# hmmlillian/Neural-Color-Transfer

Hardware: AMD Instinct MI355X
Metric: 700x700 pairs/sec end-to-end L=5->1; PatchMatch HBM GB/s vs peak (higher is better)
Workload: dtype f32

## Files before the change

### neural-color-transfer_amd/csrc/k_s1.hip

```cpp
#include "nct_internal.h"
#include "nct_device.h"
#include "nct_reduce.h"
#include <rocprim/device/device_radix_sort.hpp>
#include <rocprim/device/device_scan.hpp>

#define LAB_D(u) ((double)(u) * (1.0 / 255.0))
#define LCHK() NCT_LAUNCH_CHECK()

constexpr int S1_SEG = NCT_S1_SEG;

struct S1Sys {
    int n, h, w;
    const double *daa, *dab, *dbb;
    const double *gx, *gy;
    const int* knn_id;
    nct_s1_graph g;
    int xcd;
    int one_xcd;
};
__device__ __forceinline__ int s1_one_xcd(int bid, int sel) { return (bid & 7) == sel - 1 ? (bid >> 3) : -1; }
__device__ __forceinline__ int s1_block_of(int bid, int nblocks, int xcd) {
    if (!xcd) return bid;
    const int q = nblocks >> 3, r = nblocks & 7, x = bid & 7, idx = bid >> 3;
    return (x < r ? x * (q + 1) : r * (q + 1) + (x - r) * q) + idx;
// ... 164 lines not shown
constexpr int S1_CHUNK = 1024;
template <bool COOP>
__device__ __forceinline__ void s1_op(const S1Sys& S, const double* __restrict__ p, int i, bool live, double (&a)[3], double (&b)[3], double (&ya)[3], double (&yb)[3], int lb = -1) {
    const int w = S.w, h = S.h;
    int e0 = 0, e1 = 0, h0 = 0, h1 = 0;
#pragma unroll
    for (int c = 0; c < 3; ++c) { a[c] = 0.0; b[c] = 0.0; ya[c] = 0.0; yb[c] = 0.0; }
    if (live) {
        const int y = i / w, x = i - y * w;
        { double own[6]; ld6(p, (size_t)i, own);
#pragma unroll
          for (int c = 0; c < 3; ++c) { a[c] = own[c]; b[c] = own[3 + c]; } }
#pragma unroll
        for (int c = 0; c < 3; ++c) {
            ya[c] = S.daa[(size_t)i * 3 + c] * a[c] + S.dab[(size_t)i * 3 + c] * b[c];
            yb[c] = S.dab[(size_t)i * 3 + c] * a[c] + S.dbb[(size_t)i * 3 + c] * b[c];
        }
        auto edge = [&](int j, double wt) {
            double q[6]; ld6(p, (size_t)j, q);
#pragma unroll
            for (int c = 0; c < 3; ++c) { ya[c] += wt * (a[c] - q[c]); yb[c] += wt * (b[c] - q[3 + c]); }
        };
        {
            const bool ex[4] = {x + 1 < w, x > 0, y + 1 < h, y > 0};
            const int nj[4] = {ex[0] ? i + 1 : i, ex[1] ? i - 1 : i, ex[2] ? i + w : i, ex[3] ? i - w : i};
            const double g4[4] = {S.gx[i], S.gx[ex[1] ? i - 1 : i], S.gy[i], S.gy[ex[3] ? i - w : i]};
            double q4[4][6];
#pragma unroll
            for (int u = 0; u < 4; ++u) ld6(p, (size_t)nj[u], q4[u]);
#pragma unroll
            for (int u = 0; u < 4; ++u)
                if (ex[u]) {
                    const double wt = 2.0 * (g4[u] * g4[u]);
#pragma unroll
                    for (int c = 0; c < 3; ++c) { ya[c] += wt * (a[c] - q4[u][c]); yb[c] += wt * (b[c] - q4[u][3 + c]); }
                }
        }
#pragma unroll
        for (int k = 0; k < 8; ++k) edge(S.knn_id[(size_t)i * 8 + k], S.g.iw2[(size_t)i * 8 + k]);
        const unsigned long long s0 = S.g.starts[i], s1 = S.g.starts[i + 1];
        e0 = lo32(s0); e1 = lo32(s1); h0 = hi32(s0); h1 = hi32(s1);
    }
    if constexpr (!COOP) {
        if (live) {
            int e = e0;
            for (; e + 4 <= e1; e += 4) {
                int j[4]; double wt[4], pv[4][6];
#pragma unroll
                for (int u = 0; u < 4; ++u) { j[u] = S.g.c_src[e + u]; wt[u] = S.g.c_w[e + u]; }
#pragma unroll
                for (int u = 0; u < 4; ++u) ld6(p, (size_t)j[u], pv[u]);
#pragma unroll
                for (int u = 0; u < 4; ++u)
#pragma unroll
                    for (int c = 0; c < 3; ++c) { ya[c] += wt[u] * (a[c] - pv[u][c]); yb[c] += wt[u] * (b[c] - pv[u][3 + c]); }
            }
            for (; e < e1; ++e) {
                const int j = S.g.c_src[e]; const double wt = S.g.c_w[e];
                double q[6]; ld6(p, (size_t)j, q);
#pragma unroll
                for (int c = 0; c < 3; ++c) { ya[c] += wt * (a[c] - q[c]); yb[c] += wt * (b[c] - q[3 + c]); }
            }
        }
    } else {
        __shared__ double s_pv[6 * S1_CHUNK];
        __shared__ double s_wt[S1_CHUNK];
        const int i0 = (lb >= 0 ? lb : (int)blockIdx.x) * 256, i1 = min(i0 + 256, S.n);
        const int E0 = lo32(S.g.starts[i0]), E1 = lo32(S.g.starts[i1]);
        for (int base = E0; base < E1; base += S1_CHUNK) {
            const int cnt = min(S1_CHUNK, E1 - base);
            for (int t = threadIdx.x; t < cnt; t += 256) {
                const int j = S.g.c_src[base + t];
                s_wt[t] = S.g.c_w[base + t];
                double q[6]; ld6(p, (size_t)j, q);
#pragma unroll
                for (int c = 0; c < 6; ++c) s_pv[c * S1_CHUNK + t] = q[c];
            }
            __syncthreads();
            const int lo = max(e0, base) - base, hi = min(e1, base + cnt) - base;
            for (int t = lo; t < hi; ++t) {
                const double wt = s_wt[t];
#pragma unroll
                for (int c = 0; c < 3; ++c) { ya[c] += wt * (a[c] - s_pv[c * S1_CHUNK + t]); yb[c] += wt * (b[c] - s_pv[(3 + c) * S1_CHUNK + t]); }
            }
            __syncthreads();
        }
    }
    bool sup = false;
    if (h1 - h0 > S1_SEG) { h0 = S.g.sup_start[i]; h1 = S.g.sup_start[i + 1]; sup = true; }
    const double* __restrict__ part = sup ? S.g.sup_part : S.g.hub_part;
    for (int sg = h0; sg < h1; ++sg) {
        double q[6]; ld6(part, (size_t)sg, q);
#pragma unroll
        for (int c = 0; c < 3; ++c) { ya[c] += q[c]; yb[c] += q[3 + c]; }
    }
}

template <bool COOP>
__global__ __launch_bounds__(256) void k_s1_residual(S1Sys S, const double* __restrict__ x6, const double* __restrict__ rhs, double* __restrict__ r6) {
    const int i = blockIdx.x * 256 + threadIdx.x;
    double a[3], b[3], ya[3], yb[3];
    s1_op<COOP>(S, x6, i, i < S.n, a, b, ya, yb);
    if (i < S.n) {
        double o[6];
#pragma unroll
        for (int c = 0; c < 3; ++c) { o[c] = rhs[(size_t)i * 3 + c] - ya[c]; o[3 + c] = rhs[(size_t)(S.n + i) * 3 + c] - yb[c]; }
        st6(r6, (size_t)i, o);
    }
}
template <bool COOP>
__global__ __launch_bounds__(256) void k_s1_apply(S1Sys S, const double* __restrict__ r6, double* __restrict__ w6, double* __restrict__ partial ) {
    const int lb = S.one_xcd ? s1_one_xcd(blockIdx.x, S.one_xcd) : s1_block_of(blockIdx.x, gridDim.x, S.xcd);
    if (lb < 0) return;
    const int i = lb * 256 + threadIdx.x;
    double acc[6] = {0, 0, 0, 0, 0, 0};
    double a[3], b[3], ya[3], yb[3];
    s1_op<COOP>(S, r6, i, i < S.n, a, b, ya, yb, lb);
    if (i < S.n) {
#pragma unroll
        for (int c = 0; c < 3; ++c) {
            acc[c] = a[c] * a[c] + b[c] * b[c];
            acc[3 + c] = a[c] * ya[c] + b[c] * yb[c];
        }
        const double o[6] = {ya[0], ya[1], ya[2], yb[0], yb[1], yb[2]};
        st6(w6, (size_t)i, o);
    }
    block_reduce_store<6>(acc, partial, lb);
}

__device__ __forceinline__ void s1_scalars(bool first, const double (&sm)[6], const S1State* __restrict__ in, double tol2, S1State& o) {
#pragma unroll
    for (int c = 0; c < 3; ++c) {
        if (first) {
            const double g0 = sm[c]; const bool act = g0 > tol2;
            o.gm[c] = g0; o.be[c] = 0.0; o.al[c] = act ? g0 / sm[3 + c] : 0.0; o.active[c] = act ? 1 : 0; o.iters[c] = act ? 1 : 0;
        } else if (in->active[c]) {
            const double g1 = sm[c];
            const double be = g1 / in->gm[c];
            const double al = g1 / (sm[3 + c] - (be * g1) / in->al[c]);
            const bool act = g1 > tol2;
            o.gm[c] = g1; o.be[c] = be; o.al[c] = al; o.active[c] = act ? 1 : 0; o.iters[c] = in->iters[c] + (act ? 1 : 0);
        } else {
            o.gm[c] = in->gm[c]; o.be[c] = in->be[c]; o.al[c] = in->al[c]; o.active[c] = 0; o.iters[c] = in->iters[c];
        }
    }
}
__global__ __launch_bounds__(256) void k_s1_scal(const double* __restrict__ partial, int nb, const S1State* __restrict__ in, S1State* __restrict__ out, int first, double tol2) {
    double sm[6]; final_reduce<6>(partial, nb, sm);
    if (threadIdx.x == 0) { S1State o; s1_scalars(first != 0, sm, in, tol2, o); *out = o; }
}
constexpr int S1_FUSE_NB = 512;
template <bool FUSED>
__global__ __launch_bounds__(256) void k_s1_update(int n, int nb, const double* __restrict__ partial, const S1State* __restrict__ sin, S1State* __restrict__ sout,
                                                   int first_scal, double tol2, int first_vec, double* __restrict__ r6, const double* __restrict__ w6,
                                                   double* __restrict__ p6, double* __restrict__ s6, double* __restrict__ x6, int one_xcd) {
    const int bid = one_xcd ? s1_one_xcd(blockIdx.x, one_xcd) : (int)blockIdx.x;
    if (bid < 0) return;
    const size_t total = (size_t)3 * n;
    const size_t base = (size_t)bid * 768 + threadIdx.x;
    double2 rv[3], wv[3], pv[3], sv[3], xv[3];
    const double2* r2 = reinterpret_cast<const double2*>(r6); const double2* w2 = reinterpret_cast<const double2*>(w6);
    const double2* x2 = reinterpret_cast<const double2*>(x6); const double2* p2 = reinterpret_cast<const double2*>(p6); const double2* s2 = reinterpret_cast<const double2*>(s6);
#pragma unroll
    for (int k = 0; k < 3; ++k) {
        const size_t g0 = base + (size_t)k * 256, g = g0 < total ? g0 : total - 1;
        rv[k] = r2[g]; wv[k] = w2[g]; xv[k] = x2[g];
        pv[k] = p2[g]; sv[k] = s2[g];
        if (first_vec) { pv[k] = make_double2(0.0, 0.0); sv[k] = make_double2(0.0, 0.0); }
    }
    double al[3], be[3]; bool act[3];
    if constexpr (FUSED) {
        double sm[6]; final_reduce<6>(partial, nb, sm);
        S1State o; s1_scalars(first_scal != 0, sm, sin, tol2, o);
        if (bid == 0 && threadIdx.x == 0) *sout = o;
#pragma unroll
        for (int c = 0; c < 3; ++c) { al[c] = o.al[c]; be[c] = o.be[c]; act[c] = o.active[c] != 0; }
    } else {
#pragma unroll
        for (int c = 0; c < 3; ++c) { al[c] = sin->al[c]; be[c] = sin->be[c]; act[c] = sin->active[c] != 0; }
    }
    double2* r2o = reinterpret_cast<double2*>(r6); double2* x2o = reinterpret_cast<double2*>(x6); double2* p2o = reinterpret_cast<double2*>(p6); double2* s2o = reinterpret_cast<double2*>(s6);
#pragma unroll
    for (int k = 0; k < 3; ++k) {
        const size_t g = base + (size_t)k * 256;
        if (g >= total) continue;
        const int c0 = (int)((2 * g) % 3), c1 = (c0 + 1) % 3;
        const double a0 = c0 == 0 ? al[0] : (c0 == 1 ? al[1] : al[2]), b0 = c0 == 0 ? be[0] : (c0 == 1 ? be[1] : be[2]);
        const double a1 = c1 == 0 ? al[0] : (c1 == 1 ? al[1] : al[2]), b1 = c1 == 0 ? be[0] : (c1 == 1 ? be[1] : be[2]);
        const bool on0 = c0 == 0 ? act[0] : (c0 == 1 ? act[1] : act[2]), on1 = c1 == 0 ? act[0] : (c1 == 1 ? act[1] : act[2]);
        double2 pn, sn, xn, rn;
        pn.x = first_vec ? rv[k].x : b0 * pv[k].x + rv[k].x;  pn.y = first_vec ? rv[k].y : b1 * pv[k].y + rv[k].y;
        sn.x = first_vec ? wv[k].x : b0 * sv[k].x + wv[k].x;  sn.y = first_vec ? wv[k].y : b1 * sv[k].y + wv[k].y;
        xn.x = xv[k].x + a0 * pn.x;  xn.y = xv[k].y + a1 * pn.y;
        rn.x = rv[k].x - a0 * sn.x;  rn.y = rv[k].y - a1 * sn.y;
        if (!on0) { pn.x = pv[k].x; sn.x = sv[k].x; xn.x = xv[k].x; rn.x = rv[k].x; }
        if (!on1) { pn.y = pv[k].y; sn.y = sv[k].y; xn.y = xv[k].y; rn.y = rv[k].y; }
        if (on0 || on1) { p2o[g] = pn; s2o[g] = sn; x2o[g] = xn; r2o[g] = rn; }
    }
}
__global__ void k_pack6(int n, const double* __restrict__ x, double* __restrict__ x6) {
    const int i = blockIdx.x * blockDim.x + threadIdx.x;
    if (i >= 2 * n * 3) return;
    const int c = i % 3, part = i / (n * 3), px = (i - part * n * 3) / 3;
    x6[(size_t)px * 6 + part * 3 + c] = x[i];
}
__global__ void k_unpack6(int n, const double* __restrict__ x6, double* __restrict__ x) {
    const int i = blockIdx.x * blockDim.x + threadIdx.x;
    if (i >= 2 * n * 3) return;
    const int c = i % 3, part = i / (n * 3), px = (i - part * n * 3) / 3;
    x[i] = x6[(size_t)px * 6 + part * 3 + c];
}

int nctk_s1_solve(nct_ctx* ctx, hipStream_t s, const nct_s1_graph& g, const int* knn_id, const double* weight, float dWeight, const uint8_t* s_lab_level,
                  const uint8_t* g_lab_level, const double* gx, const double* gy, int layer, int h, int w, double* x, int* cg_iters_host ) {
    const int n = h * w, nbl = cdiv(n, 256);
    DevBuf<double> daa(ctx, (size_t)3 * n), dab(ctx, (size_t)3 * n), dbb(ctx, (size_t)3 * n), rhs(ctx, (size_t)6 * n);
    DevBuf<double> x6(ctx, (size_t)6 * n), r6(ctx, (size_t)6 * n), w6(ctx, (size_t)6 * n), p6(ctx, (size_t)6 * n), s6(ctx, (size_t)6 * n), partial(ctx, (size_t)nbl * 6);
    DevBuf<S1State> st(ctx, 2);
    if (!daa.ok() || !dab.ok() || !dbb.ok() || !rhs.ok() || !x6.ok() || !r6.ok() || !w6.ok() || !p6.ok() || !s6.ok() || !partial.ok() || !st.ok()) return NCT_ERR_HIP;
    hipLaunchKernelGGL(k_s1_setup, dim3(nbl), dim3(256), 0, s, n, weight, dWeight, s_lab_level, g_lab_level, (double*)daa, (double*)dab, (double*)dbb, (double*)rhs); LCHK();
    constexpr int one_xcd_max = 32;
    const int one_xcd = (nbl <= one_xcd_max && nbl <= S1_FUSE_NB) ? 1 + (ctx->home_xcd & 7) : 0;
    const int ogrid = one_xcd ? nbl * 8 : nbl;
    S1Sys S{n, h, w, daa, dab, dbb, gx, gy, knn_id, g, n >= 100000 ? 1 : 0, one_xcd};
    const double tol2 = 1e-6 * 1e-6;
    const int maxit = ctx->s1_maxit > 0 ? ctx->s1_maxit : (layer == 4 ? 50 : 100);
    const bool coop = n >= 100000;
    const bool fused = nbl <= S1_FUSE_NB;
    const int hub_blind = cdiv(cdiv(8 * n, S1_SEG), 4) < 256 ? cdiv(cdiv(8 * n, S1_SEG), 4) : 256;
    const int hub_grid = g.nseg_hint == 0 ? 0 : (g.nseg_hint > 0 ? (cdiv(g.nseg_hint, 4) < 4096 ? cdiv(g.nseg_hint, 4) : 4096) : hub_blind);
    const int hub2_grid = (g.nseg_hint == 0 || g.nsup_hint == 0) ? 0 : (g.nsup_hint > 0 ? (cdiv(g.nsup_hint, 4) < 1024 ? cdiv(g.nsup_hint, 4) : 1024) : (cdiv(hub_blind, S1_SEG) < 64 ? cdiv(hub_blind, S1_SEG) : 64));
    auto hub = [&](const double* v) -> int {
        if (hub_grid) { hipLaunchKernelGGL(k_s1_hub, dim3(hub_grid), dim3(256), 0, s, g, v); LCHK(); }
        if (hub2_grid) { hipLaunchKernelGGL(k_s1_hub2, dim3(hub2_grid), dim3(256), 0, s, g); LCHK(); }
        return 0;
    };
    auto apply = [&](bool kt) -> int {
        if (kt) NCT_TRY(ctx->kt_begin(s, NCT_KT_S1_APPLY));
        if (coop) hipLaunchKernelGGL(k_s1_apply<true>, dim3(nbl), dim3(256), 0, s, S, (const double*)r6, (double*)w6, (double*)partial);
        else      hipLaunchKernelGGL(k_s1_apply<false>, dim3(ogrid), dim3(256), 0, s, S, (const double*)r6, (double*)w6, (double*)partial);
        LCHK();
        if (kt) NCT_TRY(ctx->kt_end(s));
        return 0;
    };
    hipLaunchKernelGGL(k_pack6, dim3(cdiv(6 * n, 256)), dim3(256), 0, s, n, (const double*)x, (double*)x6); LCHK();
    NCT_TRY(hub(x6));
    if (coop) hipLaunchKernelGGL(k_s1_residual<true>, dim3(nbl), dim3(256), 0, s, S, (const double*)x6, (const double*)rhs, (double*)r6);
    else      hipLaunchKernelGGL(k_s1_residual<false>, dim3(nbl), dim3(256), 0, s, S, (const double*)x6, (const double*)rhs, (double*)r6);
    LCHK();
    NCT_TRY(hub(r6)); NCT_TRY(apply(false));
    S1State* slot[2] = {(S1State*)st, (S1State*)st + 1};
    for (int k = 1; k <= maxit; ++k) {
        const bool kt = ctx->kt_on && layer == 4 && k >= 3 && k < 11;
        if (fused) {
            hipLaunchKernelGGL(k_s1_update<true>, dim3(ogrid), dim3(256), 0, s, n, nbl, (const double*)partial, (const S1State*)slot[k & 1], slot[(k - 1) & 1], k == 1 ? 1 : 0, tol2,
                               k == 1 ? 1 : 0, (double*)r6, (const double*)w6, (double*)p6, (double*)s6, (double*)x6, one_xcd); LCHK();
        } else {
            if (kt) NCT_TRY(ctx->kt_begin(s, NCT_KT_S1_SCALARS));
            hipLaunchKernelGGL(k_s1_scal, dim3(1), dim3(256), 0, s, (const double*)partial, nbl, (const S1State*)slot[k & 1], slot[(k - 1) & 1], k == 1 ? 1 : 0, tol2); LCHK();
            if (kt) { NCT_TRY(ctx->kt_end(s)); NCT_TRY(ctx->kt_begin(s, NCT_KT_S1_UPDATE)); }
            hipLaunchKernelGGL(k_s1_update<false>, dim3(nbl), dim3(256), 0, s, n, nbl, (const double*)partial, (const S1State*)slot[(k - 1) & 1], slot[(k - 1) & 1], 0, tol2,
                               k == 1 ? 1 : 0, (double*)r6, (const double*)w6, (double*)p6, (double*)s6, (double*)x6, 0); LCHK();
            if (kt) NCT_TRY(ctx->kt_end(s));
        }
        if (k < maxit) { NCT_TRY(hub(r6)); NCT_TRY(apply(kt)); }
    }
    hipLaunchKernelGGL(k_unpack6, dim3(cdiv(6 * n, 256)), dim3(256), 0, s, n, (const double*)x6, x); LCHK();
    if (cg_iters_host) {
        S1State hst;
        NCT_HIP(hipMemcpyAsync(&hst, slot[(maxit - 1) & 1], sizeof hst, hipMemcpyDeviceToHost, s));
        NCT_HIP(hipStreamSynchronize(s));
        for (int c = 0; c < 3; ++c) cg_iters_host[c] = hst.iters[c];
    }
    return 0;
}
```

### neural-color-transfer_amd/csrc/k_wls_mg.hip

```cpp
#include "nct_internal.h"
#include "nct_wls_schedule.h"
#include <chrono>
#include <atomic>
#include <cstdlib>
#include <cstdio>
#include <cmath>
#include "nct_device.h"
#include <vector>
#include <cstring>
#include <string>
#include <thread>
#include <cstdarg>

namespace {
constexpr int MG_NS = 3;
static_assert(MG_NS >= 2 && MG_NS <= 4, "2, 3 or 4 smoothing sweeps per leg");
constexpr double MG_W[4] = {MG_NS == 2 ? 0.5808 : (MG_NS == 3 ? 0.5346 : 0.5193), MG_NS == 2 ? 2.6437 : (MG_NS == 3 ? 0.9677 : 0.7153), MG_NS == 3 ? 5.0974 : 1.5340, 8.0502};
constexpr double OMEGA = MG_W[0];
__host__ __device__ constexpr float mg_rk(int k) { return (float)(MG_W[k] / MG_W[0]); }
constexpr float MG_R0 = (float)(0.8 / MG_W[0]);
constexpr int NQMAX = 6;

typedef float vf;
struct Lvl { int H, W, n, nine;
// ... 716 lines not shown
                    const int i = t + k * MID_T;
                    if (i < n) {
                        vf xs; const vf y = mid_op(c[k], src, i, W, &xs);
                        const vf xv = xs + (breg[k] - y) * (c[k].dinv * mg_rk(sw));
                        dst[i] = xv;
                        if (sw == MG_NS - 1) x[k] = xv;
                    }
                }
                __syncthreads();
            }
            {
                vf* xs = (MG_NS & 1) ? sA : sB; vf* rs = (MG_NS & 1) ? sB : sA;
#pragma unroll
                for (int k = 0; k < PPT; ++k) { const int i = t + k * MID_T; if (i < n) rs[i] = breg[k] - mid_op(c[k], xs, i, W); }
            }
            __syncthreads();
            vf bc[CPT];
#pragma unroll
            for (int k = 0; k < CPT; ++k) { const int I = t + k * MID_T; bc[k] = I < C.n ? mid_restrict((MG_NS & 1) ? sB : sA, ps[k], I, C.W, W, L.H) : 0.f; }
            __syncthreads();
            asm volatile("" ::: "memory");
            mid_level<P0, D + 1>(P, q, t, sA, sB, sC, sS, bc, sweeps);
        }
        PxCoef c[PPT]; vf pw[PPT][4];
        if constexpr (D == 0) {
#pragma unroll
            for (int k = 0; k < PPT; ++k) { const int i = t + k * MID_T; if (i < n) { c[k] = px_coef<true>(L, i / W, i % W);
#pragma unroll
                for (int j = 0; j < 4; ++j) pw[k][j] = L.fpw[(size_t)j * n + i]; } }
        } else {
            if (t < n) {
                const int gy = t / W, gx = t - gy * W;
                const bool xr = gx + 1 < W, xl = gx > 0, yd = gy + 1 < L.H, yu = gy > 0;
                c[0].ex = (xr ? 1u : 0u) | (xl ? 2u : 0u) | (yd ? 4u : 0u) | (yu ? 8u : 0u) | (xr && yd ? 16u : 0u) | (xl && yd ? 32u : 0u) | (xr && yu ? 64u : 0u) | (xl && yu ? 128u : 0u);
                c[0].d = stash[t]; c[0].dinv = stash[n + t];
#pragma unroll
                for (int j = 0; j < 8; ++j) c[0].w[j] = stash[(2 + j) * n + t];
#pragma unroll
                for (int j = 0; j < 4; ++j) pw[0][j] = stash[(10 + j) * n + t];
            }
        }
#pragma unroll
        for (int k = 0; k < PPT; ++k) {
            const int i = t + k * MID_T;
            if (i < n) sA[i] = x[k] + mid_prolong(sC, pw[k], i / W, i % W, C.W, C.H);
        }
        __syncthreads();
#pragma unroll
        for (int sw = 0; sw < MG_NS; ++sw) {
            vf* src = (sw & 1) ? sB : sA; vf* dst = (sw & 1) ? sA : sB;
#pragma unroll
            for (int k = 0; k < PPT; ++k) {
                const int i = t + k * MID_T;
                if (i < n) {
                    vf xs; const vf y = mid_op(c[k], src, i, W, &xs);
                    const vf v = xs + (breg[k] - y) * (sw == 0 ? c[k].dinv : c[k].dinv * mg_rk(sw));
                    if (sw < MG_NS - 1) dst[i] = v;
                    else if (D == 0) L.x2[(size_t)q * n + i] = v; else sC[i] = v;
                }
            }
            __syncthreads();
        }
    }
}
template <int P0>
__global__ __launch_bounds__(MID_T) void k_mg_mid(const PState* __restrict__ st, MidPack P, int sweeps) {
    const int nact = st->nactive;
    __shared__ vf sA[MID_T * P0], sB[MID_T * P0], sC[MID_N1], sS[MID_STASH];
    const int q = blockIdx.x, t = threadIdx.x;
    const Lvl& L0 = P.lv[0];
    vf b[P0];
#pragma unroll
    for (int k = 0; k < P0; ++k) { const int i = t + k * MID_T; b[k] = i < L0.n ? L0.b[(size_t)q * L0.n + i] : 0.f; }
    if (nact == 0) return;
    mid_level<P0, 0>(P, q, t, sA, sB, sC, sS, b, sweeps);
}


__device__ __forceinline__ void pcg_publish(PState* __restrict__ host_out, const PState& v, int seq) {
    PState o = v; o.seq = 0;
    *host_out = o;
    __threadfence_system();
    __hip_atomic_store(&host_out->seq, seq, __ATOMIC_RELEASE, __HIP_MEMORY_SCOPE_SYSTEM);
}
template <int NQ>
__global__ __launch_bounds__(256) void k_pcg_start(Lvl L, const double* __restrict__ rough, const double* __restrict__ X , double* __restrict__ x6, double* __restrict__ r, vf* __restrict__ rf, double* __restrict__ partial) {
    const int i = blockIdx.x * 256 + threadIdx.x;
    double acc[2 * NQ];
#pragma unroll
    for (int q = 0; q < 2 * NQ; ++q) acc[q] = 0.0;
    if (i < L.n) {
        auto xv = [&](int j, int q) { return X[((size_t)(q / 3) * L.n + j) * 3 + (q % 3)]; };
        double y[NQ]; lvl_op<NQ>(L, i, xv, y);
        const double rg = rough[i];
#pragma unroll
        for (int q = 0; q < NQ; ++q) {
            const double x0 = xv(i, q);
            const double bq = rg * x0;
            const double rv = bq - y[q];
            x6[(size_t)q * L.n + i] = x0; r[(size_t)q * L.n + i] = rv; rf[(size_t)q * L.n + i] = (vf)rv;
            acc[q] = rv * rv; acc[NQ + q] = bq * bq;
        }
    }
    mg_block_reduce<2 * NQ>(acc, partial);
}
template <int NQ>
__global__ void k_pcg_start_fin(const double* __restrict__ partial, int nb, PState* __restrict__ st, double rtol2, PState* __restrict__ host_out, int seq) {
    double s[2 * NQ]; mg_final_reduce<2 * NQ>(partial, nb, s);
    if (threadIdx.x < NQ) { const int q = threadIdx.x; st->bb[q] = s[NQ + q]; st->gam[q] = 0; st->alp[q] = 0; st->iters[q] = 0; st->rho[q] = s[q];
                            st->active[q] = (s[q] > rtol2 * s[NQ + q]) ? 1 : 0; }
    __syncthreads();
    if (threadIdx.x == 0) { int na = 0; for (int q = 0; q < NQ; ++q) na += st->active[q]; st->nactive = na; if (host_out) pcg_publish(host_out, *st, seq); }
}
template <int NQ>
__global__ __launch_bounds__(256) void k_cg_apply(const PState* __restrict__ st, Lvl L, const vf* __restrict__ z, const double* __restrict__ r,
                                                  double* __restrict__ w, double* __restrict__ partial) {
    const int nact = st->nactive;
    const int lb = mg_tile_of_block(blockIdx.x, gridDim.x);
    const int i = lb * 256 + threadIdx.x;
    double acc[3 * NQ];
#pragma unroll
    for (int q = 0; q < 3 * NQ; ++q) acc[q] = 0.0;
    auto uv = [&](int j, int q) { return (double)z[(size_t)q * L.n + j]; };
    double y[NQ], rq[NQ], uq[NQ];
#pragma unroll
    for (int q = 0; q < NQ; ++q) { y[q] = 0.0; rq[q] = 0.0; uq[q] = 0.0; }
    if (i < L.n) {
        lvl_op<NQ>(L, i, uv, y);
#pragma unroll
        for (int q = 0; q < NQ; ++q) { rq[q] = r[(size_t)q * L.n + i]; uq[q] = uv(i, q); }
    }
    if (nact == 0) return;
    if (i < L.n) {
#pragma unroll
        for (int q = 0; q < NQ; ++q) {
            const double u = uq[q], rv = rq[q];
            w[(size_t)q * L.n + i] = y[q];
            acc[q] = rv * u; acc[NQ + q] = y[q] * u; acc[2 * NQ + q] = rv * rv;
        }
    }
    mg_block_reduce<3 * NQ>(acc, partial, lb);
}
template <int NQ>
__global__ void k_cg_fin(const PState* __restrict__ st, const double* __restrict__ partial, int nb, double* __restrict__ sums) {
    if (st->nactive == 0) return;
    double s[NQ]; mg_final_reduce_strided<NQ>(partial + blockIdx.x * NQ, nb, 3 * NQ, s);
    if (threadIdx.x < NQ) sums[blockIdx.x * NQ + threadIdx.x] = s[threadIdx.x];
}
template <int NQ>
__global__ __launch_bounds__(256) void k_cg_update(int n, const PState* __restrict__ sc, PState* __restrict__ sn, const double* __restrict__ sums, double rtol2, int first,
                                                   const vf* __restrict__ z, const double* __restrict__ w, double* __restrict__ p, double* __restrict__ s,
                                                   double* __restrict__ x, double* __restrict__ r, vf* __restrict__ rf, PState* __restrict__ host_out, int seq) {
    if (sc->nactive == 0) { if (blockIdx.x == 0 && threadIdx.x == 0) { *sn = *sc; if (host_out) pcg_publish(host_out, *sc, seq); } return; }
    double al[NQ], be[NQ]; bool act[NQ];
#pragma unroll
    for (int q = 0; q < NQ; ++q) {
        const double gam = sums[q], del = sums[NQ + q], rho = sums[2 * NQ + q];
        act[q] = sc->active[q] != 0 && rho > rtol2 * sc->bb[q];
        be[q] = first ? 0.0 : gam / sc->gam[q];
        al[q] = first ? gam / del : gam / (del - be[q] * gam / sc->alp[q]);
    }
    if (blockIdx.x == 0 && threadIdx.x == 0) {
        int na = 0;
#pragma unroll
        for (int q = 0; q < NQ; ++q) {
            sn->bb[q] = sc->bb[q];
            sn->gam[q] = act[q] ? sums[q] : sc->gam[q]; sn->alp[q] = act[q] ? al[q] : sc->alp[q];
            sn->iters[q] = sc->iters[q] + (act[q] ? 1 : 0); sn->active[q] = act[q] ? 1 : 0; na += act[q] ? 1 : 0;
            sn->rho[q] = sc->active[q] != 0 ? sums[2 * NQ + q] : sc->rho[q];
        }
        sn->nactive = na;
        if (host_out) pcg_publish(host_out, *sn, seq);
    }
    const int i = blockIdx.x * 256 + threadIdx.x;
    if (i >= n) return;
    vf zq[NQ]; double wq[NQ], pq[NQ], sq[NQ], xq[NQ], rq[NQ];
#pragma unroll
    for (int q = 0; q < NQ; ++q) {
        zq[q] = 0.f; wq[q] = pq[q] = sq[q] = xq[q] = rq[q] = 0.0;
        if (act[q]) {
            const size_t j = (size_t)q * n + i;
            zq[q] = z[j]; wq[q] = w[j]; xq[q] = x[j]; rq[q] = r[j];
            if (!first) { pq[q] = p[j]; sq[q] = s[j]; }
        }
    }
#pragma unroll
    for (int q = 0; q < NQ; ++q) {
        if (!act[q]) continue;
        const size_t j = (size_t)q * n + i;
        const double zv = (double)zq[q], wv = wq[q];
        const double pn = first ? zv : zv + be[q] * pq[q];
        const double sv = first ? wv : wv + be[q] * sq[q];
        p[j] = pn; s[j] = sv;
        x[j] = xq[q] + al[q] * pn;
        const double rn = rq[q] - al[q] * sv;
        r[j] = rn; rf[j] = (vf)rn;
    }
}
template <int NQ>
__global__ void k_pcg_finish(int n, const double* __restrict__ x6, double* __restrict__ X) {
    const int i = blockIdx.x * blockDim.x + threadIdx.x;
    if (i >= n * NQ) return;
    const int q = i / n, px = i - q * n;
    X[((size_t)(q / 3) * n + px) * 3 + (q % 3)] = x6[i];
}
}

#define LCHK() NCT_LAUNCH_CHECK()
namespace {
struct ErrSink {
    std::string err;
    int fail(int code, const char* fmt, ...) { char buf[512]; va_list ap; va_start(ap, fmt); vsnprintf(buf, sizeof buf, fmt, ap); va_end(ap); err = buf; return code; }
};
static std::atomic<int> g_seq{0};
struct PartBufs {
    double *x6, *r, *p, *sv, *w, *partial, *sums; PState* st;
    vf* rf;
    std::vector<Lvl> lv;
    PState* hst;
    const double* rough;
    nct_ctx* kt;
    const nct_ctx* cfg;
    int iters[NQMAX];
};
constexpr int TXB = 32, TYB = 16;
dim3 mg_grid(const Lvl& L, int tx, int ty) { return dim3(cdiv(L.W, tx) * cdiv(L.H, ty)); }
template <int NQ, bool NINE, bool X0>
void launch_down(hipStream_t s, const PState* st, const Lvl& F, const vf* b, const Lvl& C, const vf* x1) {
    constexpr int TYL = X0 ? TYB - 2 : TYB;
    if (F.n >= 100000) hipLaunchKernelGGL((k_mg_down<NQ, TXB, TYL, vf, NINE, X0>), mg_grid(F, TXB, TYL), dim3(mg_threads(TXB, TYL, X0)), 0, s, st, F, b, F.x, C, C.b, x1);
    else               hipLaunchKernelGGL((k_mg_down<NQ, 16, 8, vf, NINE, X0>), mg_grid(F, 16, 8), dim3(mg_threads(16, 8, X0)), 0, s, st, F, b, F.x, C, C.b, x1);
}
template <int NQ, bool NINE>
void launch_up(hipStream_t s, const PState* st, const Lvl& L, const vf* b, const Lvl& C) {
    if (L.n >= 100000) hipLaunchKernelGGL((k_mg_up<NQ, TXB, TYB, vf, NINE>), mg_grid(L, TXB, TYB), dim3(mg_threads(TXB, TYB)), 0, s, st, L, b, (const vf*)L.x, C.W, C.n, (const vf*)C.x2, L.x2);
    else               hipLaunchKernelGGL((k_mg_up<NQ, 16, 8, vf, NINE>), mg_grid(L, 16, 8), dim3(mg_threads(16, 8)), 0, s, st, L, b, (const vf*)L.x, C.W, C.n, (const vf*)C.x2, L.x2);
}
MidPack mid_levels(const std::vector<Lvl>& lv) {
    const int nl = (int)lv.size();
    auto mid_fits = [&](int first) {
        if (nl - first > MID_LV) return false;
        for (int l = first; l < nl; ++l) { const int d = l - first; if (lv[l].n > (d == 0 ? MID_MAXP0 * MID_T : mid_cap(d))) return false; }
        return true;
    };
    int tail0 = nl - 1;
    while (tail0 > 1 && mid_fits(tail0 - 1)) --tail0;
    MidPack pack; memset(&pack, 0, sizeof pack); pack.nl = nl - tail0;
    for (int l = tail0; l < nl; ++l) pack.lv[l - tail0] = lv[l];
    return pack;
}
int wait_published(ErrSink* ctx, hipStream_t s, const PState* slot, int want_seq) {
    const auto t0 = std::chrono::steady_clock::now();
    for (unsigned spins = 1; __atomic_load_n(&slot->seq, __ATOMIC_ACQUIRE) != want_seq; ++spins) {
        if (spins > 4096) std::this_thread::yield();
        if ((spins & 0xFFFFu) == 0) {
            const hipError_t q = hipStreamQuery(s);
            if (q != hipSuccess && q != hipErrorNotReady) return ctx->fail(NCT_ERR_HIP, "WLS MG-PCG: stream error while polling the solver state: %s", hipGetErrorString(q));
            if (std::chrono::steady_clock::now() - t0 > std::chrono::seconds(60)) return ctx->fail(NCT_ERR_HIP, "WLS MG-PCG: the solver state was not published within 60 s");
        }
    }
    return 0;
}
template <int NQ>
int pcg_part(ErrSink* ctx, hipStream_t s, double* X , PartBufs& B, double rtol) {
    const std::vector<Lvl>& lv = B.lv;
    const Lvl& F = lv[0];
    const int N = F.n, nb = cdiv(N, 256);
    const PState* cur = B.st;
    const double rtol2 = rtol * rtol;
    const bool lines = B.cfg->wls_lines != 0;
    hipLaunchKernelGGL(k_pcg_start<NQ>, dim3(nb), dim3(256), 0, s, F, B.rough, (const double*)X, B.x6, B.r, B.rf, B.partial); LCHK();
    int seq_of_slot[2] = {++g_seq, 0};
    hipLaunchKernelGGL(k_pcg_start_fin<NQ>, dim3(1), dim3(256), 0, s, (const double*)B.partial, nb, B.st, rtol2, &B.hst[0], seq_of_slot[0]); LCHK();
    auto down = [&](int l) {
        if (l == 0 && lines) launch_down<NQ, false, true>(s, cur, lv[0], B.rf, lv[1], lv[0].x2);
        else if (l == 0)       launch_down<NQ, false, false>(s, cur, lv[0], B.rf, lv[1], nullptr);
        else                   launch_down<NQ, true, false>(s, cur, lv[l], lv[l].b, lv[l + 1], nullptr);
    };
    auto block_step = [&](bool post) {
        const dim3 gl(cdiv(lv[0].W, LBX) * cdiv(lv[0].H, LBY));
        if (!post) hipLaunchKernelGGL((k_mg_block<NQ, false>), gl, dim3(LBX * LBY), 0, s, cur, lv[0], (const vf*)B.rf, (const vf*)nullptr, lv[0].x2);
        else       hipLaunchKernelGGL((k_mg_block<NQ, true>), gl, dim3(LBX * LBY), 0, s, cur, lv[0], (const vf*)B.rf, (const vf*)lv[0].x2, lv[0].x);
    };
    auto up = [&](int l) {
        if (l == 0) launch_up<NQ, false>(s, cur, lv[0], B.rf, lv[1]);
        else        launch_up<NQ, true>(s, cur, lv[l], lv[l].b, lv[l + 1]);
    };
    const MidPack pack = mid_levels(lv);
    const int tail0 = (int)lv.size() - pack.nl;
    bool ktime = false;
    auto kt_b = [&](int id) -> int { if (ktime && B.kt->kt_begin(s, id)) return ctx->fail(NCT_ERR_HIP, "%s", B.kt->err.c_str()); return 0; };
    auto kt_e = [&]() -> int { if (ktime && B.kt->kt_end(s)) return ctx->fail(NCT_ERR_HIP, "%s", B.kt->err.c_str()); return 0; };
    auto vcycle = [&]() -> int {
        if (lines) { NCT_TRY(kt_b(NCT_KT_WLS_BLOCK_PRE)); block_step(false); LCHK(); NCT_TRY(kt_e()); }
        NCT_TRY(kt_b(NCT_KT_WLS_DOWN)); down(0); LCHK(); NCT_TRY(kt_e());
        NCT_TRY(kt_b(NCT_KT_WLS_COARSE));
        for (int l = 1; l < tail0; ++l) { down(l); LCHK(); }
        if (lv[tail0].n <= MID_T) hipLaunchKernelGGL(k_mg_mid<1>, dim3(NQ), dim3(MID_T), 0, s, cur, pack, 60);
        else                      hipLaunchKernelGGL(k_mg_mid<2>, dim3(NQ), dim3(MID_T), 0, s, cur, pack, 60);
        LCHK();
        for (int l = tail0 - 1; l >= 1; --l) { up(l); LCHK(); }
        NCT_TRY(kt_e());
        NCT_TRY(kt_b(NCT_KT_WLS_UP)); up(0); LCHK(); NCT_TRY(kt_e());
        if (lines) { NCT_TRY(kt_b(NCT_KT_WLS_BLOCK_POST)); block_step(true); LCHK(); NCT_TRY(kt_e()); }
        return 0;
    };
    const vf* z = lines ? lv[0].x : lv[0].x2;
    auto iteration = [&](int it, PState* pub_to, int pub_seq) -> int {
        cur = B.st + (it & 1);
        PState* nxt = B.st + ((it + 1) & 1);
        ktime = B.kt != nullptr && it >= 2 && it < 6;
        NCT_TRY(vcycle());
        NCT_TRY(kt_b(NCT_KT_WLS_APPLY));
        hipLaunchKernelGGL(k_cg_apply<NQ>, dim3(nb), dim3(256), 0, s, cur, F, z, (const double*)B.r, B.w, B.partial); LCHK();
        NCT_TRY(kt_e());
        hipLaunchKernelGGL(k_cg_fin<NQ>, dim3(3), dim3(256), 0, s, cur, (const double*)B.partial, nb, B.sums); LCHK();
        NCT_TRY(kt_b(NCT_KT_WLS_UPDATE));
        hipLaunchKernelGGL(k_cg_update<NQ>, dim3(nb), dim3(256), 0, s, N, cur, nxt, (const double*)B.sums, rtol2, it == 0 ? 1 : 0, z, (const double*)B.w,
                           B.p, B.sv, B.x6, B.r, B.rf, pub_to, pub_seq); LCHK();
        NCT_TRY(kt_e());
        cur = nxt;
        return 0;
    };
    WlsSchedule sched{NQ, B.cfg->wls_maxit, B.cfg->wls_forecast != 0, rtol2};
    while (true) {
        const int want = sched.next_batch(), pub = (sched.issued + 1) & 1;
        for (int k = 0; k < want; ++k) {
            const bool last = k == want - 1;
            if (last) seq_of_slot[pub] = ++g_seq;
            NCT_TRY(iteration(sched.it + k, last ? &B.hst[pub] : nullptr, last ? seq_of_slot[pub] : 0));
        }
        sched.enqueued(want);
        if (!sched.pending()) break;
        const int slot = (sched.seen + 1) & 1;
        NCT_TRY(wait_published(ctx, s, &B.hst[slot], seq_of_slot[slot]));
        if (sched.read(B.hst[slot])) break;
    }
    if (!sched.done) return ctx->fail(NCT_ERR_HIP, "WLS MG-PCG did not converge in %d iterations", B.cfg->wls_maxit);
    hipLaunchKernelGGL(k_pcg_finish<NQ>, dim3(cdiv(N * NQ, 256)), dim3(256), 0, s, N, (const double*)B.x6, X); LCHK();
    int mx = 0;
    for (int q = 0; q < NQ; ++q) { B.iters[q] = sched.iters[q]; mx = B.iters[q] > mx ? B.iters[q] : mx; }
    if (B.cfg->wls_trace)
        fprintf(stderr, "nct wls: %d x %d, %d iterations enqueued, %d needed (+1 that finds every system converged), %d snapshots read\n", F.W, F.H, sched.it, mx, sched.seen + 1);
    return 0;
}
struct SolveBlocks {
    nct_ctx* c; std::vector<void*> owned; bool failed = false;
// ... 103 lines not shown
```

Measured before the change: 15.94.

## Defer CG solution updates to every other iteration to cut x traffic

The pipelined CG update kernels in the S1 solver and the WLS multigrid PCG now read and write the solution vector x only on every second iteration. On those iterations they apply the previous step's pending alpha*p contribution together with the current one. The last iteration also skips the p, s and r stores and the w load, since those values are never used again. This removes roughly half the x load and store traffic from a bandwidth-bound update. The cost is more bookkeeping logic and a correctness dependence on the parity and flush handling, especially when a channel converges on an odd iteration.

```diff
diff --git a/neural-color-transfer_amd/csrc/k_s1.hip b/neural-color-transfer_amd/csrc/k_s1.hip
--- a/neural-color-transfer_amd/csrc/k_s1.hip
+++ b/neural-color-transfer_amd/csrc/k_s1.hip
@@ -340,8 +340,9 @@
 constexpr int S1_FUSE_NB = 512;
 template <bool FUSED>
 __global__ __launch_bounds__(256) void k_s1_update(int n, int nb, const double* __restrict__ partial, const S1State* __restrict__ sin, S1State* __restrict__ sout,
-                                                   int first_scal, double tol2, int first_vec, double* __restrict__ r6, const double* __restrict__ w6,
-                                                   double* __restrict__ p6, double* __restrict__ s6, double* __restrict__ x6, int one_xcd) {
+                                                   int first_scal, double tol2, int first_vec, int carry, const S1State* __restrict__ pend, int last,
+                                                   double* __restrict__ r6, const double* __restrict__ w6, double* __restrict__ p6, double* __restrict__ s6,
+                                                   double* __restrict__ x6, int one_xcd) {
     const int bid = one_xcd ? s1_one_xcd(blockIdx.x, one_xcd) : (int)blockIdx.x;
     if (bid < 0) return;
     const size_t total = (size_t)3 * n;
@@ -352,11 +353,18 @@
 #pragma unroll
     for (int k = 0; k < 3; ++k) {
         const size_t g0 = base + (size_t)k * 256, g = g0 < total ? g0 : total - 1;
-        rv[k] = r2[g]; wv[k] = w2[g]; xv[k] = x2[g];
-        pv[k] = p2[g]; sv[k] = s2[g];
-        if (first_vec) { pv[k] = make_double2(0.0, 0.0); sv[k] = make_double2(0.0, 0.0); }
+        const double2 zero = make_double2(0.0, 0.0);
+        rv[k] = r2[g]; wv[k] = zero; xv[k] = zero; pv[k] = zero; sv[k] = zero;
+        if (carry) xv[k] = x2[g];
+        if (!first_vec) pv[k] = p2[g];
+        if (!last) { wv[k] = w2[g]; if (!first_vec) sv[k] = s2[g]; }
     }
     double al[3], be[3]; bool act[3];
+    double alp[3] = {0.0, 0.0, 0.0}; bool pnd[3] = {false, false, false};
+    if (pend) {
+#pragma unroll
+        for (int c = 0; c < 3; ++c) { alp[c] = pend->al[c]; pnd[c] = pend->active[c] != 0; }
+    }
     if constexpr (FUSED) {
         double sm[6]; final_reduce<6>(partial, nb, sm);
         S1State o; s1_scalars(first_scal != 0, sm, sin, tol2, o);
@@ -376,14 +384,19 @@
         const double a0 = c0 == 0 ? al[0] : (c0 == 1 ? al[1] : al[2]), b0 = c0 == 0 ? be[0] : (c0 == 1 ? be[1] : be[2]);
         const double a1 = c1 == 0 ? al[0] : (c1 == 1 ? al[1] : al[2]), b1 = c1 == 0 ? be[0] : (c1 == 1 ? be[1] : be[2]);
         const bool on0 = c0 == 0 ? act[0] : (c0 == 1 ? act[1] : act[2]), on1 = c1 == 0 ? act[0] : (c1 == 1 ? act[1] : act[2]);
-        double2 pn, sn, xn, rn;
+        const double q0 = c0 == 0 ? alp[0] : (c0 == 1 ? alp[1] : alp[2]), q1 = c1 == 0 ? alp[0] : (c1 == 1 ? alp[1] : alp[2]);
+        const bool pe0 = c0 == 0 ? pnd[0] : (c0 == 1 ? pnd[1] : pnd[2]), pe1 = c1 == 0 ? pnd[0] : (c1 == 1 ? pnd[1] : pnd[2]);
+        double2 pn, sn, xn, rn, xm = xv[k];
+        if (pe0) xm.x = xv[k].x + q0 * pv[k].x;
+        if (pe1) xm.y = xv[k].y + q1 * pv[k].y;
         pn.x = first_vec ? rv[k].x : b0 * pv[k].x + rv[k].x;  pn.y = first_vec ? rv[k].y : b1 * pv[k].y + rv[k].y;
         sn.x = first_vec ? wv[k].x : b0 * sv[k].x + wv[k].x;  sn.y = first_vec ? wv[k].y : b1 * sv[k].y + wv[k].y;
-        xn.x = xv[k].x + a0 * pn.x;  xn.y = xv[k].y + a1 * pn.y;
+        xn.x = xm.x + a0 * pn.x;  xn.y = xm.y + a1 * pn.y;
         rn.x = rv[k].x - a0 * sn.x;  rn.y = rv[k].y - a1 * sn.y;
-        if (!on0) { pn.x = pv[k].x; sn.x = sv[k].x; xn.x = xv[k].x; rn.x = rv[k].x; }
-        if (!on1) { pn.y = pv[k].y; sn.y = sv[k].y; xn.y = xv[k].y; rn.y = rv[k].y; }
-        if (on0 || on1) { p2o[g] = pn; s2o[g] = sn; x2o[g] = xn; r2o[g] = rn; }
+        if (!on0) { pn.x = pv[k].x; sn.x = sv[k].x; xn.x = xm.x; rn.x = rv[k].x; }
+        if (!on1) { pn.y = pv[k].y; sn.y = sv[k].y; xn.y = xm.y; rn.y = rv[k].y; }
+        if (carry && (on0 || on1 || pe0 || pe1)) x2o[g] = xn;
+        if (!last && (on0 || on1)) { p2o[g] = pn; s2o[g] = sn; r2o[g] = rn; }
     }
 }
 __global__ void k_pack6(int n, const double* __restrict__ x, double* __restrict__ x6) {
@@ -440,15 +453,17 @@
     S1State* slot[2] = {(S1State*)st, (S1State*)st + 1};
     for (int k = 1; k <= maxit; ++k) {
         const bool kt = ctx->kt_on && layer == 4 && k >= 3 && k < 11;
+        const int last = k == maxit ? 1 : 0, carry = (k % 2 == 0 || last) ? 1 : 0;
+        const S1State* pend = k % 2 == 0 ? slot[k & 1] : nullptr;
         if (fused) {
             hipLaunchKernelGGL(k_s1_update<true>, dim3(ogrid), dim3(256), 0, s, n, nbl, (const double*)partial, (const S1State*)slot[k & 1], slot[(k - 1) & 1], k == 1 ? 1 : 0, tol2,
-                               k == 1 ? 1 : 0, (double*)r6, (const double*)w6, (double*)p6, (double*)s6, (double*)x6, one_xcd); LCHK();
+                               k == 1 ? 1 : 0, carry, pend, last, (double*)r6, (const double*)w6, (double*)p6, (double*)s6, (double*)x6, one_xcd); LCHK();
         } else {
             if (kt) NCT_TRY(ctx->kt_begin(s, NCT_KT_S1_SCALARS));
             hipLaunchKernelGGL(k_s1_scal, dim3(1), dim3(256), 0, s, (const double*)partial, nbl, (const S1State*)slot[k & 1], slot[(k - 1) & 1], k == 1 ? 1 : 0, tol2); LCHK();
             if (kt) { NCT_TRY(ctx->kt_end(s)); NCT_TRY(ctx->kt_begin(s, NCT_KT_S1_UPDATE)); }
             hipLaunchKernelGGL(k_s1_update<false>, dim3(nbl), dim3(256), 0, s, n, nbl, (const double*)partial, (const S1State*)slot[(k - 1) & 1], slot[(k - 1) & 1], 0, tol2,
-                               k == 1 ? 1 : 0, (double*)r6, (const double*)w6, (double*)p6, (double*)s6, (double*)x6, 0); LCHK();
+                               k == 1 ? 1 : 0, carry, pend, last, (double*)r6, (const double*)w6, (double*)p6, (double*)s6, (double*)x6, 0); LCHK();
             if (kt) NCT_TRY(ctx->kt_end(s));
         }
         if (k < maxit) { NCT_TRY(hub(r6)); NCT_TRY(apply(kt)); }
diff --git a/neural-color-transfer_amd/csrc/k_wls_mg.hip b/neural-color-transfer_amd/csrc/k_wls_mg.hip
--- a/neural-color-transfer_amd/csrc/k_wls_mg.hip
+++ b/neural-color-transfer_amd/csrc/k_wls_mg.hip
@@ -892,13 +892,15 @@
                                                    const vf* __restrict__ z, const double* __restrict__ w, double* __restrict__ p, double* __restrict__ s,
                                                    double* __restrict__ x, double* __restrict__ r, vf* __restrict__ rf, PState* __restrict__ host_out, int seq) {
     if (sc->nactive == 0) { if (blockIdx.x == 0 && threadIdx.x == 0) { *sn = *sc; if (host_out) pcg_publish(host_out, *sc, seq); } return; }
-    double al[NQ], be[NQ]; bool act[NQ];
+    double al[NQ], be[NQ], pal[NQ]; bool act[NQ], carry[NQ], flush[NQ];
 #pragma unroll
     for (int q = 0; q < NQ; ++q) {
         const double gam = sums[q], del = sums[NQ + q], rho = sums[2 * NQ + q];
         act[q] = sc->active[q] != 0 && rho > rtol2 * sc->bb[q];
         be[q] = first ? 0.0 : gam / sc->gam[q];
         al[q] = first ? gam / del : gam / (del - be[q] * gam / sc->alp[q]);
+        const bool odd = (sc->iters[q] & 1) != 0;
+        pal[q] = sc->alp[q]; carry[q] = act[q] && odd; flush[q] = sc->active[q] != 0 && !act[q] && odd;
     }
     if (blockIdx.x == 0 && threadIdx.x == 0) {
         int na = 0;
@@ -918,21 +920,23 @@
 #pragma unroll
     for (int q = 0; q < NQ; ++q) {
         zq[q] = 0.f; wq[q] = pq[q] = sq[q] = xq[q] = rq[q] = 0.0;
+        const size_t j = (size_t)q * n + i;
         if (act[q]) {
-            const size_t j = (size_t)q * n + i;
-            zq[q] = z[j]; wq[q] = w[j]; xq[q] = x[j]; rq[q] = r[j];
+            zq[q] = z[j]; wq[q] = w[j]; rq[q] = r[j];
+            if (carry[q]) xq[q] = x[j];
             if (!first) { pq[q] = p[j]; sq[q] = s[j]; }
-        }
+        } else if (flush[q]) { xq[q] = x[j]; pq[q] = p[j]; }
     }
 #pragma unroll
     for (int q = 0; q < NQ; ++q) {
+        const size_t j = (size_t)q * n + i;
+        if (flush[q]) x[j] = xq[q] + pal[q] * pq[q];
         if (!act[q]) continue;
-        const size_t j = (size_t)q * n + i;
         const double zv = (double)zq[q], wv = wq[q];
         const double pn = first ? zv : zv + be[q] * pq[q];
         const double sv = first ? wv : wv + be[q] * sq[q];
         p[j] = pn; s[j] = sv;
-        x[j] = xq[q] + al[q] * pn;
+        if (carry[q]) { const double xm = xq[q] + pal[q] * pq[q]; x[j] = xm + al[q] * pn; }
         const double rn = rq[q] - al[q] * sv;
         r[j] = rn; rf[j] = (vf)rn;
     }
```

Result: no change. 16.06 (median of 6 runs) (+0.7%).
